# apache/arrow

Measured on AMD Instinct MI355X. Metric: filter_take_mrows_per_s, higher is better.
Workload: dtype int64; 1 GPU; Filter+Take int64[1000000000] + validity (10% null), boolean mask 10% true, FilterOptions::DROP; take indices = the mask's row numbers (monotonic; indices_nonzero: uint64 through CallFunction, GetTakeIndices: uint32 in the mirror), no boundscheck; inputs = splitmix64 streams of SURVEY.md 8(d) (seeds 1,2,3); rows=1000000000, selected_rows=99992053, parallelism=single-gpu

## Files before the change

arrow_amd/csrc/selection.hip:

```cpp
#include "arx_common.h"

#include <string.h>

#include <algorithm>
#include <type_traits>

namespace arx {

struct FilterWsHeader {
  int64_t total;
  int64_t ntiles;
  int64_t ngroups;
  int64_t length;
  int64_t valid;
  int64_t pad[3];
};
static_assert(sizeof(FilterWsHeader) == 64, "header is one 64-byte line");

struct FilterWsView {
  FilterWsHeader* hdr;
  int64_t* group_excl;
  int64_t* group_total;
  uint32_t* tile_counts;
  int64_t* group_valid;
};

static inline int64_t num_tiles(int64_t length) { return ceil_div(length, kTileRows); }
static inline int64_t num_groups(int64_t length) {
  return ceil_div(num_tiles(length), kTilesPerGroup);
}

static inline FilterWsView ws_view(void* ws, int64_t length) {
  FilterWsView v;
  const int64_t ng = num_groups(length);
  uint8_t* p = static_cast<uint8_t*>(ws);
  v.hdr = reinterpret_cast<FilterWsHeader*>(p);
  v.group_excl = reinterpret_cast<int64_t*>(p + 64);
  v.group_total = v.group_excl + ng;
  v.tile_counts = reinterpret_cast<uint32_t*>(v.group_total + ng);
  v.group_valid = reinterpret_cast<int64_t*>(v.tile_counts + ng * kTilesPerGroup);
  return v;
}

__device__ __forceinline__ uint64_t emit_word(const Bits& mask, const Bits& mvalid, int64_t w,
                                              bool emit_null, bool invert,
                                              uint64_t* mask_valid_out) {
  uint64_t m = load_word(mask, w);
  const uint64_t mv = load_word(mvalid, w);
  *mask_valid_out = mv;
  if (emit_null || invert) {
    const uint64_t in_range = load_word(Bits{nullptr, 0, mask.length, 0}, w);
    if (invert) m = ~m & in_range;
    if (emit_null) return (m | ~mv) & in_range;
  }
  return m & mv;
}

template <bool VALID>
__global__ __launch_bounds__(kBlock) void count_kernel(Bits mask, Bits mvalid, Bits vvalid, int emit_null,
                                                       int invert, int64_t ntiles,
                                                       uint32_t* tile_counts,
                                                       int64_t* group_total, int64_t* group_valid) {
  __shared__ uint32_t wave_sums[kWavesPerBlock];
  __shared__ uint32_t wave_valid[kWavesPerBlock];
  const int lane = lane_id();
  const int wave = threadIdx.x >> 6;
  const int64_t group = blockIdx.x;
  const int64_t t0 = group * kTilesPerGroup + wave * 16;
  uint32_t mine = 0;
  uint32_t kv = 0;
#pragma unroll 4
  for (int i = 0; i < 16; ++i) {
    const int64_t t = t0 + i;
    uint32_t k = 0;
    if (t < ntiles) {
      uint64_t mv;
      const uint64_t e = emit_word(mask, mvalid, t * 64 + lane, emit_null != 0, invert != 0, &mv);
      k = __popcll(e);
      if constexpr (VALID) kv += __popcll(e & mv & load_word(vvalid, t * 64 + lane));
    }
    const uint32_t s = wave_reduce_sum_u32(k);
    if (lane == i) mine = s;
  }
  if (lane < 16) tile_counts[t0 + lane] = mine;
  const uint32_t wsum = wave_reduce_sum_u32(lane < 16 ? mine : 0u);
  if (lane == 0) wave_sums[wave] = wsum;
  if constexpr (VALID) {
    const uint32_t vsum = wave_reduce_sum_u32(kv);
    if (lane == 0) wave_valid[wave] = vsum;
  }
  __syncthreads();
  if (threadIdx.x == 0) {
    int64_t s = 0, v = 0;
    for (int i = 0; i < kWavesPerBlock; ++i) {
      s += wave_sums[i];
      if constexpr (VALID) v += wave_valid[i];
    }
    group_total[group] = s;
    if constexpr (VALID) group_valid[group] = v;
  }
}

__global__ __launch_bounds__(1024) void scan_kernel(const int64_t* group_total, int64_t ngroups,
                                                    int64_t* group_excl, FilterWsHeader* hdr,
                                                    const int64_t* group_valid = nullptr) {
  __shared__ int64_t wave_tot[16];
  __shared__ int64_t carry_s;
  __shared__ unsigned long long valid_s;
  const int tid = threadIdx.x;
  const int lane = tid & 63;
  const int wave = tid >> 6;
  if (tid == 0) carry_s = 0;
  if (tid == 0) valid_s = 0;
  __syncthreads();
  if (group_valid != nullptr) {
    int64_t mine = 0;
    for (int64_t i = tid; i < ngroups; i += 1024) mine += group_valid[i];
#pragma unroll
    for (int d = 32; d >= 1; d >>= 1) mine += __shfl_xor(mine, d, 64);
    if (lane == 0 && mine != 0) atomicAdd(&valid_s, static_cast<unsigned long long>(mine));
    __syncthreads();
  }
  for (int64_t base = 0; base < ngroups; base += 1024) {
    const int64_t i = base + tid;
    const int64_t v = i < ngroups ? group_total[i] : 0;
    int64_t x = v;
#pragma unroll
    for (int d = 1; d < 64; d <<= 1) {
      const int64_t n = __shfl_up(x, d, 64);
      if (lane >= d) x += n;
    }
    if (lane == 63) wave_tot[wave] = x;
    __syncthreads();
    int64_t wave_prefix = 0;
    for (int k = 0; k < wave; ++k) wave_prefix += wave_tot[k];
    const int64_t carry = carry_s;
    if (i < ngroups) group_excl[i] = carry + wave_prefix + x - v;
    __syncthreads();
    if (tid == 1023) carry_s = carry + wave_prefix + x;
    __syncthreads();
  }
  if (tid == 0) {
    hdr->total = carry_s;
    hdr->valid = static_cast<int64_t>(valid_s);
  }
}

struct CompactArgs {
  const uint8_t* values;
  Bits mask;
  Bits mvalid;
  Bits vvalid;
  int64_t length;
  int64_t ntiles;
  const uint32_t* tile_counts;
  const int64_t* group_excl;
  uint8_t* out_data;
  uint64_t* out_validity;
  int emit_null;
  int invert;
  int values_aligned16;
};

constexpr int kFlushBytes = 2048;

template <int RING>
struct __attribute__((aligned(16))) CompactLds {
  uint8_t ring[kWavesPerBlock][RING];
  uint64_t vbits[kWavesPerBlock][72];
};

template <int W>
struct ElemT;
template <> struct ElemT<1> { using type = uint8_t; };
template <> struct ElemT<2> { using type = uint16_t; };
template <> struct ElemT<4> { using type = uint32_t; };
template <> struct ElemT<8> { using type = uint64_t; };
template <> struct ElemT<16> { using type = uint4; };
struct Elem32 { uint4 lo, hi; };
template <> struct ElemT<32> { using type = Elem32; };

template <int W>
__device__ __forceinline__ typename ElemT<W>::type zero_elem() {
  if constexpr (W == 32) {
    return Elem32{make_uint4(0, 0, 0, 0), make_uint4(0, 0, 0, 0)};
  } else if constexpr (W == 16) {
    return make_uint4(0, 0, 0, 0);
  } else {
    return 0;
  }
}

constexpr int kSelNt = 3;

template <int W>
__device__ __forceinline__ typename ElemT<W>::type sel_load(const typename ElemT<W>::type* p, bool nt) {
  using E = typename ElemT<W>::type;
  if constexpr (W == 32) {
    return *p;
  } else if constexpr (W == 16) {
    return nt ? nt_load16(p) : *p;
  } else {
    return nt ? nt_load<E>(p) : *p;
  }
}
template <int W>
__device__ __forceinline__ void sel_store(typename ElemT<W>::type* p, typename ElemT<W>::type v) {
  using E = typename ElemT<W>::type;
  if constexpr (W == 32) {
    *p = v;
  } else if constexpr (W == 16) {
    if constexpr ((kSelNt & 2) != 0) nt_store16(p, v); else *p = v;
  } else {
    if constexpr ((kSelNt & 2) != 0) nt_store<E>(p, v); else *p = v;
  }
}

__device__ __forceinline__ void wave_lds_sync() {
  __builtin_amdgcn_fence(__ATOMIC_RELEASE, "wavefront");
  __builtin_amdgcn_wave_barrier();
  __builtin_amdgcn_fence(__ATOMIC_ACQUIRE, "wavefront");
}

template <int W, int RING>
__device__ __forceinline__ void flush_region(const uint8_t* ring, uint8_t* gbase, int64_t F,
                                             int64_t lo, int64_t hi, int lane) {
  using E = typename ElemT<W>::type;
  constexpr int R = 16 / W;
  const int ring_off = static_cast<int>(F & (RING - 1));
#pragma unroll
  for (int h = 0; h < kFlushBytes / (16 * kWave); ++h) {
    const int g = h * kWave + lane;
    const int64_t gs = F + g * 16;
    const int64_t ge = gs + 16;
    if (ge <= lo || gs >= hi) continue;
    const uint8_t* src = ring + ring_off + g * 16;
    uint8_t* dst = gbase + gs;
    if (gs >= lo && ge <= hi) {
      sel_store<16>(reinterpret_cast<uint4*>(dst), *reinterpret_cast<const uint4*>(src));
    } else {
#pragma unroll
      for (int e = 0; e < R; ++e) {
        const int64_t es = gs + e * W;
        if (es >= lo && es + W <= hi) {
          *reinterpret_cast<E*>(dst + e * W) = *reinterpret_cast<const E*>(src + e * W);
        }
      }
    }
  }
}

template <int W, int B>
struct Batch {
  using E = typename ElemT<W>::type;
  static constexpr int R = 16 / W;
  uint32_t bits[B];
  uint32_t zbits[B];
  uint32_t rank[B];
  E v[B][R];
};

template <int R, bool EMIT>
__device__ __forceinline__ void select_words(uint64_t Ew, uint32_t p, uint64_t Zw,
                                             int widx_base, int lane, uint64_t* wE, uint32_t* wp,
                                             uint64_t* wZ) {
  constexpr int kLanesPerWord = 64 / R;
  const int q_mine = lane / kLanesPerWord;
  uint64_t e = 0, z = 0;
  uint32_t pp = 0;
#pragma unroll
  for (int q = 0; q < R; ++q) {
    const int src = widx_base + q;
    const uint32_t lo = __builtin_amdgcn_readlane(static_cast<uint32_t>(Ew), src);
    const uint32_t hi = __builtin_amdgcn_readlane(static_cast<uint32_t>(Ew >> 32), src);
    const uint32_t pq = __builtin_amdgcn_readlane(p, src);
    uint64_t zq = 0;
    if constexpr (EMIT) {
      const uint32_t zlo = __builtin_amdgcn_readlane(static_cast<uint32_t>(Zw), src);
      const uint32_t zhi = __builtin_amdgcn_readlane(static_cast<uint32_t>(Zw >> 32), src);
      zq = (static_cast<uint64_t>(zhi) << 32) | zlo;
    }
    if (q == q_mine) {
      e = (static_cast<uint64_t>(hi) << 32) | lo;
      pp = pq;
      z = zq;
    }
  }
  *wE = e;
  *wp = pp;
  *wZ = z;
}

struct TileCtx {
  uint64_t Ew, Zw;
  uint32_t p;
  int lane;
  int64_t tile_row0;
  const uint8_t* values;
  __amdgpu_buffer_rsrc_t rsrc;
};

template <int W, bool IOTA, bool EMIT, bool ALIGNED, int B>
__device__ __forceinline__ void issue_batch(const TileCtx& c, int j0, Batch<W, B>& b) {
  using E = typename ElemT<W>::type;
  constexpr int R = 16 / W;
  constexpr int kRowsPerIter = kWave * R;
#pragma unroll
  for (int i = 0; i < B; ++i) {
    const int j = j0 + i;
    const int row_in_tile = j * kRowsPerIter + c.lane * R;
    const int bpos = row_in_tile & 63;
    uint64_t wE, wZ;
    uint32_t wp;
    select_words<R, EMIT>(c.Ew, c.p, c.Zw, j * R, c.lane, &wE, &wp, &wZ);
    b.bits[i] = static_cast<uint32_t>(wE >> bpos) & ((1u << R) - 1u);
    b.zbits[i] = static_cast<uint32_t>(wZ >> bpos) & ((1u << R) - 1u);
    b.rank[i] = wp + __popcll(wE & low_mask64(bpos));
    if constexpr (IOTA) {
#pragma unroll
      for (int r = 0; r < R; ++r) b.v[i][r] = static_cast<E>(c.tile_row0 + row_in_tile + r);
    } else {
      const int64_t row = c.tile_row0 + row_in_tile;
      const uint8_t* src = c.values + row * static_cast<int64_t>(W);
      if constexpr (ALIGNED) {
        const uint32_t voff = b.bits[i] != 0 ? static_cast<uint32_t>(row_in_tile * W) : kBufferSkip;
        const uint4 q = (kSelNt & 1) ? buffer_load_b128_nt(c.rsrc, voff) : buffer_load_b128(c.rsrc, voff);
        if constexpr (W == 16) {
          b.v[i][0] = q;
        } else {
          const E* qe = reinterpret_cast<const E*>(&q);
#pragma unroll
          for (int r = 0; r < R; ++r) b.v[i][r] = qe[r];
        }
      } else {
#pragma unroll
        for (int r = 0; r < R; ++r) {
          b.v[i][r] = zero_elem<W>();
          if ((b.bits[i] >> r) & 1u) {
            if constexpr (W == 16) {
              const uint64_t* s64 = reinterpret_cast<const uint64_t*>(src + r * W);
              const uint64_t lo64 = s64[0], hi64 = s64[1];
              b.v[i][r] = make_uint4(static_cast<uint32_t>(lo64), static_cast<uint32_t>(lo64 >> 32),
                                     static_cast<uint32_t>(hi64), static_cast<uint32_t>(hi64 >> 32));
            } else {
              b.v[i][r] = *reinterpret_cast<const E*>(src + r * W);
            }
          }
        }
      }
    }
  }
}

template <int W, int B, int RING>
__device__ __forceinline__ void consume_batch(const Batch<W, B>& b, uint8_t* ring, int64_t a0) {
  using E = typename ElemT<W>::type;
  constexpr int R = 16 / W;
#pragma unroll
  for (int i = 0; i < B; ++i) {
    if (b.bits[i] != 0) {
      uint32_t rk = b.rank[i];
#pragma unroll
      for (int r = 0; r < R; ++r) {
        if ((b.bits[i] >> r) & 1u) {
          E e = b.v[i][r];
          if ((b.zbits[i] >> r) & 1u) e = zero_elem<W>();
          const int ro = static_cast<int>((a0 + static_cast<int64_t>(rk) * W) & (RING - 1));
          *reinterpret_cast<E*>(ring + ro) = e;
          ++rk;
        }
      }
    }
  }
}

template <int W, bool IOTA, bool EMIT, bool ALIGNED, int B, bool PIPE>
__global__ __launch_bounds__(kBlock) void compact_kernel(CompactArgs a) {
  using E = typename ElemT<W>::type;
  constexpr int R = 16 / W;
  constexpr int kRowsPerIter = kWave * R;
  constexpr int kIters = kTileRows / kRowsPerIter;
  constexpr int kWordsPerIter = kRowsPerIter / 64;
  constexpr int kBatches = kIters / B;
  constexpr int RING = (B <= 2) ? 4096 : 8192;
  static_assert(kIters % B == 0, "batch must divide the iteration count");
  static_assert(!PIPE || kBatches % 2 == 0, "pipelined form walks the batches in pairs");

  __shared__ CompactLds<RING> lds;

  const int lane = lane_id();
  const int wave = __builtin_amdgcn_readfirstlane(threadIdx.x >> 6);
  const int64_t t = static_cast<int64_t>(blockIdx.x) * kWavesPerBlock + wave;
  if (t >= a.ntiles) return;

  const int64_t w = t * 64 + lane;
  uint64_t mv;
  const uint64_t Ew = emit_word(a.mask, a.mvalid, w, EMIT, a.invert != 0, &mv);
  const uint32_t k = __popcll(Ew);
  const uint32_t incl = wave_inclusive_scan_u32(k);
  const uint32_t p = incl - k;
  const uint32_t total = __shfl(incl, 63, 64);
  if (total == 0) return;

  const int64_t grp = t >> 6;
  const int tin = static_cast<int>(t & 63);
  const uint32_t cprev = lane < tin ? a.tile_counts[grp * kTilesPerGroup + lane] : 0u;
  const int64_t off = a.group_excl[grp] + wave_reduce_sum_u32(cprev);

  uint8_t* ring = lds.ring[wave];
  const int64_t a0 =
      static_cast<int64_t>((reinterpret_cast<uint64_t>(a.out_data) + static_cast<uint64_t>(off) * W) &
                           (kFlushBytes - 1));
  uint8_t* gbase = a.out_data + (off * static_cast<int64_t>(W) - a0);
  int64_t flushed = 0;

  TileCtx c;
  c.Ew = Ew;
  c.Zw = EMIT ? (Ew & ~mv) : 0;
  c.p = p;
  c.lane = lane;
  c.tile_row0 = t * kTileRows;
  c.values = a.values;
  c.rsrc = make_rsrc(IOTA ? nullptr : a.values + c.tile_row0 * static_cast<int64_t>(W),
                     static_cast<uint32_t>(kTileRows * W));

  auto flush_check = [&](int next_batch) {
    const uint32_t cum = next_batch < kBatches
                             ? __builtin_amdgcn_readlane(p, next_batch * B * kWordsPerIter)
                             : total;
    const int64_t written = a0 + static_cast<int64_t>(cum) * W;
    if (written - flushed >= kFlushBytes) {
      wave_lds_sync();
      while (written - flushed >= kFlushBytes) {
        flush_region<W, RING>(ring, gbase, flushed, a0, written, lane);
        flushed += kFlushBytes;
      }
      wave_lds_sync();
    }
  };

  bool tile_done = false;
  if constexpr (IOTA) {
    if (a0 + static_cast<int64_t>(total) * W <= RING) {
      uint64_t m = Ew;
      uint32_t rk = p;
      while (m != 0) {
        const int bpos = __ffsll(static_cast<unsigned long long>(m)) - 1;
// ... 317 lines not shown
      }
    }
    E val[U];
#pragma unroll
    for (int u = 0; u < U; ++u) {
      const E* src = ok[u] ? (values + idx[u]) : (out + pos[u]);
      val[u] = sel_load<W>(src, (kSelNt & 4) != 0);
    }
    if constexpr (HAS_SV) {
      uint8_t vb[U];
#pragma unroll
      for (int u = 0; u < U; ++u) {
        const uint64_t bit = ok[u] ? static_cast<uint64_t>(a.src_valid_offset) + idx[u] : 0;
        vb[u] = a.src_valid_bytes[bit >> 3];
      }
#pragma unroll
      for (int u = 0; u < U; ++u) {
        const uint64_t bit = static_cast<uint64_t>(a.src_valid_offset) + idx[u];
        ok[u] = ok[u] && ((vb[u] >> (bit & 7)) & 1);
      }
    }
#pragma unroll
    for (int u = 0; u < U; ++u) {
      const int64_t p = base + u * 64 + lane;
      if (p <= last) sel_store<W>(out + p, ok[u] ? val[u] : zero_elem<W>());
      const uint64_t vbal = __ballot(ok[u]);
      nvalid += __popcll(vbal);
      if (a.out_validity != nullptr && lane == 0 && (base + u * 64) <= last) {
        a.out_validity[(base >> 6) + u] = vbal;
      }
    }
  }
  if (a.valid_count != nullptr && lane == 0 && nvalid != 0) atomicAdd(a.valid_count, nvalid);
}

template <int UB> struct RowUnit;
template <> struct RowUnit<1> { typedef uint8_t type; };
template <> struct RowUnit<2> { typedef uint16_t type; };
template <> struct RowUnit<4> { typedef uint32_t type; };
template <> struct RowUnit<8> { typedef uint64_t type; };
template <> struct RowUnit<16> { typedef arx_u32x4 type; };

template <int UB, typename IdxT, bool HAS_IV, bool HAS_SV>
__global__ __launch_bounds__(kBlock) void take_rows_kernel(TakeArgs a, uint32_t units_per_row) {
  using E = typename RowUnit<UB>::type;
  const int lane = lane_id();
  const int64_t nwaves = static_cast<int64_t>(gridDim.x) * kWavesPerBlock;
  const int64_t wave_g = static_cast<int64_t>(blockIdx.x) * kWavesPerBlock + __builtin_amdgcn_readfirstlane(threadIdx.x >> 6);
  const int64_t nchunks = (a.length + 63) >> 6;
  const int64_t last = a.length - 1;
  const IdxT* __restrict__ indices = reinterpret_cast<const IdxT*>(a.indices);
  const E* __restrict__ values = reinterpret_cast<const E*>(a.values);
  E* __restrict__ out = reinterpret_cast<E*>(a.out_data);
  uint64_t nvalid = 0;
  for (int64_t c = wave_g; c < nchunks; c += nwaves) {
    const int64_t base = c << 6;
    const int64_t p = base + lane <= last ? base + lane : last;
    uint64_t idx = static_cast<uint64_t>(indices[p]);
    bool ok = base + lane <= last;
    if constexpr (HAS_IV) ok = ok && ((load_word_nb(a.ivalid, base >> 6) >> lane) & 1ull);
    if constexpr (HAS_SV) {
      const uint64_t bit = ok ? static_cast<uint64_t>(a.src_valid_offset) + idx : 0;
      ok = ok && ((a.src_valid_bytes[bit >> 3] >> (bit & 7)) & 1);
    }
    if (!ok) idx = 0;
    const uint64_t vbal = __ballot(ok);
    nvalid += __popcll(vbal);
    if (a.out_validity != nullptr && lane == 0) a.out_validity[base >> 6] = vbal;
    const int rows_here = static_cast<int>(last - base + 1 < 64 ? last - base + 1 : 64);
    const uint32_t total = static_cast<uint32_t>(rows_here) * units_per_row;
    const uint32_t idx_lo = static_cast<uint32_t>(idx), idx_hi = static_cast<uint32_t>(idx >> 32);
    for (uint32_t t = lane; t < ((total + 63u) & ~63u); t += 64) {
      const uint32_t tt = t < total ? t : total - 1;
      const uint32_t row = tt / units_per_row;
      const uint32_t j = tt - row * units_per_row;
      const uint64_t src = (static_cast<uint64_t>(__shfl(idx_hi, static_cast<int>(row), 64)) << 32) | __shfl(idx_lo, static_cast<int>(row), 64);
      const bool row_ok = (vbal >> row) & 1ull;
      E v = E{};
      if (row_ok) v = values[src * units_per_row + j];
      if (t < total) out[(static_cast<uint64_t>(base) + row) * units_per_row + j] = v;
    }
  }
  if (a.valid_count != nullptr && lane == 0 && nvalid != 0) atomicAdd(a.valid_count, nvalid);
}

constexpr int kTakeMaxCols = 16;
struct TakeColsArgs {
  const uint8_t* values[kTakeMaxCols];
  const uint8_t* src_valid_bytes[kTakeMaxCols];
  int64_t src_valid_offset[kTakeMaxCols];
  uint8_t* out_data[kTakeMaxCols];
  uint64_t* out_validity[kTakeMaxCols];
  int width[kTakeMaxCols];
  int num_cols;
  const uint8_t* indices;
  Bits ivalid;
  int64_t length;
  unsigned long long* valid_counts;
};

template <int W, int U>
__device__ __forceinline__ uint64_t take_one_column(const TakeColsArgs& a, int c, const int64_t (&pos)[U],
                                                    const uint64_t (&idx)[U], const bool (&ok0)[U], int64_t base,
                                                    int64_t last, int lane) {
  using E = typename ElemT<W>::type;
  const E* __restrict__ values = reinterpret_cast<const E*>(a.values[c]);
  E* __restrict__ out = reinterpret_cast<E*>(a.out_data[c]);
  const uint8_t* __restrict__ svb = a.src_valid_bytes[c];
  const uint64_t svo = static_cast<uint64_t>(a.src_valid_offset[c]);
  E val[U];
  bool ok[U];
#pragma unroll
  for (int u = 0; u < U; ++u) {
    const E* src = ok0[u] ? (values + idx[u]) : (out + pos[u]);
    val[u] = *src;
    ok[u] = ok0[u];
  }
  if (svb != nullptr) {
    uint8_t vb[U];
#pragma unroll
    for (int u = 0; u < U; ++u) vb[u] = svb[(ok0[u] ? svo + idx[u] : 0) >> 3];
#pragma unroll
    for (int u = 0; u < U; ++u) ok[u] = ok[u] && ((vb[u] >> ((svo + idx[u]) & 7)) & 1);
  }
  uint64_t nvalid = 0;
#pragma unroll
  for (int u = 0; u < U; ++u) {
    const int64_t p = base + u * 64 + lane;
    if (p <= last) out[p] = ok[u] ? val[u] : zero_elem<W>();
    const uint64_t vbal = __ballot(ok[u]);
    nvalid += __popcll(vbal);
    if (a.out_validity[c] != nullptr && lane == 0 && (base + u * 64) <= last) a.out_validity[c][(base >> 6) + u] = vbal;
  }
  return nvalid;
}

template <typename IdxT, bool HAS_IV>
__global__ __launch_bounds__(kBlock) void take_columns_kernel(TakeColsArgs a) {
  constexpr int U = 4;
  const int lane = lane_id();
  const int64_t nwaves = static_cast<int64_t>(gridDim.x) * kWavesPerBlock;
  const int64_t wave_g = static_cast<int64_t>(blockIdx.x) * kWavesPerBlock +
                         __builtin_amdgcn_readfirstlane(threadIdx.x >> 6);
  const int64_t nchunks = (a.length + 64 * U - 1) / (64 * U);
  const int64_t last = a.length - 1;
  const IdxT* __restrict__ indices = reinterpret_cast<const IdxT*>(a.indices);
  uint64_t nvalid[kTakeMaxCols];
  for (int c = 0; c < kTakeMaxCols; ++c) nvalid[c] = 0;
  for (int64_t ch = wave_g; ch < nchunks; ch += nwaves) {
    const int64_t base = ch * (64 * U);
    int64_t pos[U];
    uint64_t idx[U];
    bool ok0[U];
#pragma unroll
    for (int u = 0; u < U; ++u) {
      const int64_t p = base + u * 64 + lane;
      pos[u] = p <= last ? p : last;
      idx[u] = static_cast<uint64_t>(indices[pos[u]]);
    }
#pragma unroll
    for (int u = 0; u < U; ++u) {
      ok0[u] = (base + u * 64 + lane) <= last;
      if constexpr (HAS_IV) {
        const uint64_t wbits = load_word_nb(a.ivalid, (base >> 6) + u);
        ok0[u] = ok0[u] && ((wbits >> lane) & 1ull);
      }
    }
    for (int c = 0; c < a.num_cols; ++c) {
      uint64_t nv;
      switch (a.width[c]) {
        case 1: nv = take_one_column<1, U>(a, c, pos, idx, ok0, base, last, lane); break;
        case 2: nv = take_one_column<2, U>(a, c, pos, idx, ok0, base, last, lane); break;
        case 4: nv = take_one_column<4, U>(a, c, pos, idx, ok0, base, last, lane); break;
        case 8: nv = take_one_column<8, U>(a, c, pos, idx, ok0, base, last, lane); break;
        case 16: nv = take_one_column<16, U>(a, c, pos, idx, ok0, base, last, lane); break;
        default: nv = take_one_column<32, U>(a, c, pos, idx, ok0, base, last, lane); break;
      }
      nvalid[c] += nv;
    }
  }
  if (a.valid_counts != nullptr && lane == 0) {
    for (int c = 0; c < a.num_cols; ++c) {
      if (nvalid[c] != 0) atomicAdd(a.valid_counts + c, nvalid[c]);
    }
  }
}

template <typename IdxT>
__global__ __launch_bounds__(kBlock) void take_bits_kernel(TakeArgs a, int64_t value_bit_offset) {
  const int lane = lane_id();
  const int64_t nwaves = static_cast<int64_t>(gridDim.x) * kWavesPerBlock;
  const int64_t wave_g = static_cast<int64_t>(blockIdx.x) * kWavesPerBlock +
                         __builtin_amdgcn_readfirstlane(threadIdx.x >> 6);
  const int64_t nwords = (a.length + 63) >> 6;
  const int64_t last = a.length - 1;
  const IdxT* __restrict__ indices = reinterpret_cast<const IdxT*>(a.indices);
  uint64_t* __restrict__ out = reinterpret_cast<uint64_t*>(a.out_data);
  uint64_t nvalid = 0;
  for (int64_t w = wave_g; w < nwords; w += nwaves) {
    const int64_t p = (w << 6) + lane;
    const int64_t pc = p <= last ? p : last;
    const uint64_t idx = static_cast<uint64_t>(indices[pc]);
    bool ok = p <= last && ((load_word(a.ivalid, w) >> lane) & 1ull);
    if (ok && a.src_valid_bytes != nullptr) {
      const uint64_t vb = static_cast<uint64_t>(a.src_valid_offset) + idx;
      ok = (a.src_valid_bytes[vb >> 3] >> (vb & 7)) & 1;
    }
    bool bit = false;
    if (ok) {
      const uint64_t b = static_cast<uint64_t>(value_bit_offset) + idx;
      bit = (a.values[b >> 3] >> (b & 7)) & 1;
    }
    const uint64_t data_bal = __ballot(bit);
    const uint64_t valid_bal = __ballot(ok);
    nvalid += __popcll(valid_bal);
    if (lane == 0) {
      out[w] = data_bal;
      if (a.out_validity != nullptr) a.out_validity[w] = valid_bal;
    }
  }
  if (a.valid_count != nullptr && lane == 0 && nvalid != 0) atomicAdd(a.valid_count, nvalid);
}

struct BoundsWs {
  unsigned long long first_bad_pos;
  long long bad_value_signed;
  unsigned long long bad_value_unsigned;
  int64_t pad[5];
};

template <typename IdxT>
__global__ __launch_bounds__(kBlock) void bounds_kernel(const uint8_t* indices, Bits ivalid,
                                                        int64_t length, uint64_t upper,
                                                        BoundsWs* ws) {
  const int64_t stride = static_cast<int64_t>(gridDim.x) * blockDim.x;
  unsigned long long bad = ~0ull;
  for (int64_t i = static_cast<int64_t>(blockIdx.x) * blockDim.x + threadIdx.x; i < length;
       i += stride) {
    const IdxT v = reinterpret_cast<const IdxT*>(indices)[i];
    const bool valid = (load_word(ivalid, i >> 6) >> (i & 63)) & 1ull;
    bool oob;
    if constexpr (std::is_signed<IdxT>::value) {
      oob = v < 0 || static_cast<uint64_t>(v) >= upper;
    } else {
      oob = static_cast<uint64_t>(v) >= upper;
    }
    if (valid && oob) {
      bad = static_cast<unsigned long long>(i);
      break;
    }
  }
  if (bad != ~0ull) atomicMin(&ws->first_bad_pos, bad);
}

template <typename IdxT>
__global__ void bounds_fetch_kernel(const uint8_t* indices, BoundsWs* ws) {
  const unsigned long long pos = ws->first_bad_pos;
  if (pos == ~0ull) return;
  const IdxT v = reinterpret_cast<const IdxT*>(indices)[pos];
  ws->bad_value_signed = static_cast<long long>(v);
  ws->bad_value_unsigned = static_cast<unsigned long long>(v);
}

static int check_mask(const ArxSpan* mask, int null_selection) {
  if (mask == nullptr) {
    set_error("filter mask is NULL");
    return ARX_INVALID;
  }
  if (mask->length < 0 || mask->offset < 0) {
    set_error("negative length/offset");
    return ARX_INVALID;
  }
  if (mask->length > 0 && mask->data == nullptr) {
    set_error("filter mask has no data buffer");
    return ARX_INVALID;
  }
  if (null_selection != ARX_FILTER_DROP && null_selection != ARX_FILTER_EMIT_NULL) {
    set_error("bad null_selection %d", null_selection);
    return ARX_INVALID;
  }
  return ARX_OK;
}

static inline const void* effective_validity(const ArxSpan* s) {
  return (s->null_count != 0) ? s->validity : nullptr;
}

static int launch_count(const ArxSpan* mask, int null_selection, void* ws, size_t ws_bytes,
                        hipStream_t st, int invert = 0, const ArxSpan* values = nullptr) {
  const int rc = check_mask(mask, null_selection);
  if (rc != ARX_OK) return rc;
  const size_t need = arx_filter_workspace_bytes(mask->length);
  if (ws == nullptr || ws_bytes < need) {
    set_error("filter workspace too small: %zu < %zu", ws_bytes, need);
    return ARX_INVALID;
  }
  if ((reinterpret_cast<uint64_t>(ws) & 63) != 0) {
    set_error("filter workspace must be 64-byte aligned");
    return ARX_INVALID;
  }
  FilterWsView v = ws_view(ws, mask->length);
  const int64_t nt = num_tiles(mask->length);
  const int64_t ng = num_groups(mask->length);
  FilterWsHeader h{};
  h.total = 0;
  h.ntiles = nt;
  h.ngroups = ng;
  h.length = mask->length;
  ARX_HIP(hipMemcpyAsync(v.hdr, &h, sizeof(h), hipMemcpyHostToDevice, st));
  if (mask->length == 0) return ARX_OK;
  const Bits mb = make_bits(mask->data, mask->offset, mask->length);
  const Bits mvb = make_bits(effective_validity(mask), mask->offset, mask->length);
  if (values != nullptr) {
    const Bits vvb = make_bits(effective_validity(values), values->offset, mask->length);
    hipLaunchKernelGGL((count_kernel<true>), dim3(static_cast<unsigned>(ng)), dim3(kBlock), 0, st, mb, mvb, vvb,
                       null_selection, invert, nt, v.tile_counts, v.group_total, v.group_valid);
    ARX_CHECK_LAUNCH("count_kernel");
    hipLaunchKernelGGL(scan_kernel, dim3(1), dim3(1024), 0, st, v.group_total, ng, v.group_excl, v.hdr,
                       static_cast<const int64_t*>(v.group_valid));
  } else {
    hipLaunchKernelGGL((count_kernel<false>), dim3(static_cast<unsigned>(ng)), dim3(kBlock), 0, st, mb, mvb, mvb,
                       null_selection, invert, nt, v.tile_counts, v.group_total, static_cast<int64_t*>(nullptr));
    ARX_CHECK_LAUNCH("count_kernel");
    hipLaunchKernelGGL(scan_kernel, dim3(1), dim3(1024), 0, st, v.group_total, ng, v.group_excl, v.hdr,
                       static_cast<const int64_t*>(nullptr));
  }
  ARX_CHECK_LAUNCH("scan_kernel");
  return ARX_OK;
}

static Knob<int> g_filter_batch{4};
static Knob<int> g_filter_pipe{1};
static Knob<int> g_filter_sparse{-1};
static const KnobRow kSelectionKnobs[] = {
    {"filter_batch", g_filter_batch, knob_snap_down<1, 4>},
    {"filter_pipe", g_filter_pipe, knob_bool},
    {"filter_sparse", g_filter_sparse, knob_tri},
};
KnobTable selection_knobs() { return knob_table(kSelectionKnobs); }

template <int W, bool IOTA, bool EMIT, bool ALIGNED>
static void launch_compact_e(const CompactArgs& a, unsigned grid, hipStream_t st) {
  constexpr int kIters = kTileRows / (kWave * (16 / W));
  constexpr int kBig = kIters >= 8 ? 4 : 2;
  if (ALIGNED && g_filter_batch >= 4 && g_filter_pipe) {
    hipLaunchKernelGGL((compact_kernel<W, IOTA, EMIT, ALIGNED, kBig, true>), dim3(grid),
                       dim3(kBlock), 0, st, a);
  } else {
    hipLaunchKernelGGL((compact_kernel<W, IOTA, EMIT, ALIGNED, 1, false>), dim3(grid), dim3(kBlock),
                       0, st, a);
  }
}

template <int W, bool IOTA>
static void launch_compact_w(const CompactArgs& a, unsigned grid, hipStream_t st) {
  const bool aligned = IOTA || a.values_aligned16 != 0;
  if (a.emit_null) {
    if (aligned) launch_compact_e<W, IOTA, true, true>(a, grid, st);
    else if constexpr (!IOTA) launch_compact_e<W, IOTA, true, false>(a, grid, st);
  } else {
    if (aligned) launch_compact_e<W, IOTA, false, true>(a, grid, st);
    else if constexpr (!IOTA) launch_compact_e<W, IOTA, false, false>(a, grid, st);
  }
}

template <int W, bool IOTA = false>
static void launch_sparse_w(const CompactArgs& a, unsigned grid, hipStream_t st) {
  if (a.emit_null) {
    hipLaunchKernelGGL((compact_sparse_kernel<W, true, IOTA>), dim3(grid), dim3(kBlock), 0, st, a);
  } else {
    hipLaunchKernelGGL((compact_sparse_kernel<W, false, IOTA>), dim3(grid), dim3(kBlock), 0, st, a);
  }
}

static int launch_compact(bool iota, int W, const CompactArgs& a, hipStream_t st,
                          int64_t out_length = -1) {
  const unsigned grid = static_cast<unsigned>(ceil_div(a.ntiles, kWavesPerBlock));
  const int filter_sparse = g_filter_sparse;
  const bool sparse = !iota && !a.invert &&
                      (filter_sparse == 1 ||
                       (filter_sparse < 0 &&
                        (W >= 8 || (out_length >= 0 && out_length * 4 <= a.length))));
  if (iota && !a.invert && filter_sparse != 0 && (W == 2 || W == 4 || W == 8)) {
    if (W == 2) launch_sparse_w<2, true>(a, grid, st);
    else if (W == 4) launch_sparse_w<4, true>(a, grid, st);
    else launch_sparse_w<8, true>(a, grid, st);
    ARX_CHECK_LAUNCH("compact_sparse_kernel<IOTA>");
    return ARX_OK;
  }
  if (sparse) {
    switch (W) {
      case 1: launch_sparse_w<1>(a, grid, st); break;
      case 2: launch_sparse_w<2>(a, grid, st); break;
      case 4: launch_sparse_w<4>(a, grid, st); break;
      case 8: launch_sparse_w<8>(a, grid, st); break;
      case 16: launch_sparse_w<16>(a, grid, st); break;
      case 32: launch_sparse_w<32>(a, grid, st); break;
      default:
        set_error("unsupported byte width %d for the gfx950 filter", W);
        return ARX_NOT_IMPLEMENTED;
    }
    ARX_CHECK_LAUNCH("compact_sparse_kernel");
    return ARX_OK;
  }
  if (iota) {
    switch (W) {
      case 2: launch_compact_w<2, true>(a, grid, st); break;
      case 4: launch_compact_w<4, true>(a, grid, st); break;
      default:
        set_error("unsupported index width %d", W);
        return ARX_NOT_IMPLEMENTED;
    }
  } else {
    switch (W) {
      case 1: launch_compact_w<1, false>(a, grid, st); break;
      case 2: launch_compact_w<2, false>(a, grid, st); break;
      case 4: launch_compact_w<4, false>(a, grid, st); break;
      case 8: launch_compact_w<8, false>(a, grid, st); break;
      case 16: launch_compact_w<16, false>(a, grid, st); break;
      default:
        set_error("unsupported byte width %d for the gfx950 filter", W);
        return ARX_NOT_IMPLEMENTED;
    }
  }
  ARX_CHECK_LAUNCH("compact_kernel");
  return ARX_OK;
}

static int zero_out_validity(void* out_validity, int64_t out_length, hipStream_t st) {
  if (out_validity == nullptr) return ARX_OK;
  if ((reinterpret_cast<uint64_t>(out_validity) & 7) != 0) {
    set_error("out_validity must be 8-byte aligned");
    return ARX_INVALID;
  }
  if (out_length < 0) {
    set_error("out_length (from arx_filter_count) is required when out_validity is given");
    return ARX_INVALID;
  }
  if (out_length > 0) {
    ARX_HIP(hipMemsetAsync(out_validity, 0, static_cast<size_t>(ceil_div(out_length, 64)) * 8, st));
  }
  return ARX_OK;
}

size_t selection_workspace_bytes(int64_t length) { return arx_filter_workspace_bytes(length); }

int selection_bit_positions(const void* bitmap, int64_t bit_offset, int64_t length, bool invert,
                            void* ws, size_t ws_bytes, uint32_t* out, int64_t* out_count_host,
                            hipStream_t st) {
  ArxSpan m{};
  m.validity = nullptr;
  m.data = bitmap;
  m.offset = bit_offset;
  m.length = length;
  m.null_count = 0;
  int rc = launch_count(&m, ARX_FILTER_DROP, ws, ws_bytes, st, invert ? 1 : 0);
  if (rc != ARX_OK) return rc;
  int64_t total = 0;
  ARX_HIP(hipMemcpyAsync(&total, ws, sizeof(int64_t), hipMemcpyDeviceToHost, st));
  ARX_HIP(hipStreamSynchronize(st));
  *out_count_host = total;
  if (total == 0) return ARX_OK;
  FilterWsView v = ws_view(ws, length);
  CompactArgs a{};
  a.values = nullptr;
  a.mask = make_bits(bitmap, bit_offset, length);
  a.mvalid = make_bits(nullptr, 0, length);
  a.vvalid = make_bits(nullptr, 0, length);
  a.length = length;
  a.ntiles = num_tiles(length);
  a.tile_counts = v.tile_counts;
  a.group_excl = v.group_excl;
  a.out_data = reinterpret_cast<uint8_t*>(out);
  a.out_validity = nullptr;
  a.emit_null = 0;
  a.invert = invert ? 1 : 0;
  a.values_aligned16 = 1;
  return launch_compact(true, 4, a, st);
}

}

using namespace arx;

extern "C" {

size_t arx_filter_workspace_bytes(int64_t length) {
  if (length < 0) length = 0;
  const int64_t ng = num_groups(length);
  return static_cast<size_t>(64 + ng * 16 + ng * kTilesPerGroup * 4 + ng * 8 + 64);
}

int arx_filter_count_async(const ArxSpan* mask, int null_selection, void* ws, size_t ws_bytes,
                           void* stream) {
  return launch_count(mask, null_selection, ws, ws_bytes, as_stream(stream));
}

int arx_filter_count_nulls(const ArxSpan* values, const ArxSpan* mask, int null_selection, void* ws, size_t ws_bytes,
                           int64_t* out_length, int64_t* out_null_count, void* stream) {
  if (out_length == nullptr || out_null_count == nullptr || values == nullptr) {
    set_error("values / out_length / out_null_count is NULL");
    return ARX_INVALID;
  }
  if (mask != nullptr && values->length != mask->length) {
    set_error("filter values and mask differ in length (%lld vs %lld)", static_cast<long long>(values->length),
              static_cast<long long>(mask->length));
    return ARX_INVALID;
  }
  hipStream_t st = as_stream(stream);
  const int rc = launch_count(mask, null_selection, ws, ws_bytes, st, 0, values);
  if (rc != ARX_OK) return rc;
  int64_t hdr[5] = {0, 0, 0, 0, 0};
  ARX_HIP(hipMemcpyAsync(hdr, ws, sizeof(hdr), hipMemcpyDeviceToHost, st));
  ARX_HIP(hipStreamSynchronize(st));
  *out_length = hdr[0];
  *out_null_count = mask->length == 0 ? 0 : hdr[0] - hdr[4];
  return ARX_OK;
}

int arx_filter_count(const ArxSpan* mask, int null_selection, void* ws, size_t ws_bytes,
                     int64_t* out_length, void* stream) {
  if (out_length == nullptr) {
    set_error("out_length is NULL");
    return ARX_INVALID;
  }
  hipStream_t st = as_stream(stream);
  const int rc = launch_count(mask, null_selection, ws, ws_bytes, st);
  if (rc != ARX_OK) return rc;
  int64_t total = 0;
  ARX_HIP(hipMemcpyAsync(&total, ws, sizeof(int64_t), hipMemcpyDeviceToHost, st));
  ARX_HIP(hipStreamSynchronize(st));
  *out_length = total;
  return ARX_OK;
}

int arx_filter_exec(const ArxSpan* values, int byte_width, const ArxSpan* mask, int null_selection,
                    const void* ws, int64_t out_length, void* out_data, void* out_validity,
                    void* stream) {
  int rc = check_mask(mask, null_selection);
  if (rc != ARX_OK) return rc;
  if (values == nullptr || ws == nullptr) {
    set_error("values/ws is NULL");
    return ARX_INVALID;
  }
  if (values->length != mask->length) {
    set_error("Array arguments must all be the same length (values %lld vs filter %lld)",
              static_cast<long long>(values->length), static_cast<long long>(mask->length));
    return ARX_INVALID;
  }
  if (mask->length == 0) return ARX_OK;
  if (values->data == nullptr || out_data == nullptr) {
    set_error("values/out data buffer is NULL");
    return ARX_INVALID;
  }
  hipStream_t st = as_stream(stream);
  FilterWsView v = ws_view(const_cast<void*>(ws), mask->length);
  CompactArgs a{};
  a.values = static_cast<const uint8_t*>(values->data) + values->offset * byte_width;
  a.mask = make_bits(mask->data, mask->offset, mask->length);
  a.mvalid = make_bits(effective_validity(mask), mask->offset, mask->length);
  a.vvalid = make_bits(effective_validity(values), values->offset, values->length);
  a.length = mask->length;
  a.ntiles = num_tiles(mask->length);
  a.tile_counts = v.tile_counts;
  a.group_excl = v.group_excl;
  a.out_data = static_cast<uint8_t*>(out_data);
  a.out_validity = static_cast<uint64_t*>(out_validity);
  a.emit_null = null_selection == ARX_FILTER_EMIT_NULL && a.mvalid.base != nullptr;
  a.values_aligned16 = (reinterpret_cast<uint64_t>(a.values) & 15) == 0;
  if ((reinterpret_cast<uint64_t>(out_data) % byte_width) != 0) {
    set_error("out_data is not aligned to the element width");
    return ARX_INVALID;
  }
  rc = zero_out_validity(out_validity, out_length, st);
  if (rc != ARX_OK) return rc;
  return launch_compact(false, byte_width, a, st, out_length);
}

int arx_expand_by_mask(const void* dense, int byte_width, const ArxSpan* mask, const void* ws, void* out_data,
                       void* stream) {
  int rc = check_mask(mask, ARX_FILTER_DROP);
  if (rc != ARX_OK) return rc;
  if (ws == nullptr) {
    set_error("ws is NULL (run arx_filter_count on the mask first)");
    return ARX_INVALID;
  }
  if (mask->length == 0) return ARX_OK;
  if (out_data == nullptr || (reinterpret_cast<uint64_t>(out_data) % byte_width) != 0 ||
      (dense != nullptr && (reinterpret_cast<uint64_t>(dense) % byte_width) != 0)) {
    set_error("expand: NULL or misaligned buffer");
    return ARX_INVALID;
  }
  FilterWsView v = ws_view(const_cast<void*>(ws), mask->length);
  CompactArgs a{};
  a.values = static_cast<const uint8_t*>(dense);
  a.mask = make_bits(mask->data, mask->offset, mask->length);
  a.mvalid = make_bits(effective_validity(mask), mask->offset, mask->length);
  a.length = mask->length;
  a.ntiles = num_tiles(mask->length);
  a.tile_counts = v.tile_counts;
  a.group_excl = v.group_excl;
  a.out_data = static_cast<uint8_t*>(out_data);
  const unsigned grid = static_cast<unsigned>(ceil_div(a.ntiles, kWavesPerBlock));
  hipStream_t st = as_stream(stream);
  switch (byte_width) {
    case 1: hipLaunchKernelGGL((expand_kernel<1>), dim3(grid), dim3(kBlock), 0, st, a); break;
    case 2: hipLaunchKernelGGL((expand_kernel<2>), dim3(grid), dim3(kBlock), 0, st, a); break;
    case 4: hipLaunchKernelGGL((expand_kernel<4>), dim3(grid), dim3(kBlock), 0, st, a); break;
    case 8: hipLaunchKernelGGL((expand_kernel<8>), dim3(grid), dim3(kBlock), 0, st, a); break;
    case 16: hipLaunchKernelGGL((expand_kernel<16>), dim3(grid), dim3(kBlock), 0, st, a); break;
    default:
      set_error("unsupported byte width %d for expand", byte_width);
      return ARX_NOT_IMPLEMENTED;
  }
  ARX_CHECK_LAUNCH("expand_kernel");
  return ARX_OK;
}

int arx_mask_to_indices(const ArxSpan* mask, int null_selection, const void* ws, int64_t out_length,
                        int index_width, void* out_indices, void* out_validity, void* stream) {
  int rc = check_mask(mask, null_selection);
  if (rc != ARX_OK) return rc;
  if (ws == nullptr) {
    set_error("ws is NULL");
    return ARX_INVALID;
  }
  if (index_width != 2 && index_width != 4 && index_width != 8) {
    set_error("index_width must be 2, 4 or 8");
// ... 389 lines not shown
```

Measured before the change: 291,300 Mrows/s.

## Batch count-kernel bitmap loads up front and drop host header memcpy

The count kernel now issues every bitmap word load for a wave's 16 tiles up front into registers, using an aligned fast path when no shifts are present and a shifted two-word path otherwise. It falls back to per-word loads near the buffer end. It also packs two tile popcounts into a single wave reduction, and adds a launch-bounds occupancy hint. The host-to-device header memcpy is removed; the scan kernel now writes the full header itself, which saves an async copy on the stream. The cost is higher register pressure from the preloaded arrays.

After: 293,900 Mrows/s, median of 6. Within noise of the previous version (+0.9%).

```diff
diff --git a/arrow_amd/csrc/selection.hip b/arrow_amd/csrc/selection.hip
--- a/arrow_amd/csrc/selection.hip
+++ b/arrow_amd/csrc/selection.hip
@@ -42,25 +42,92 @@
   return v;
 }
 
+__device__ __forceinline__ uint64_t emit_combine(int64_t length, int64_t w, uint64_t m, uint64_t mv,
+                                                 bool emit_null, bool invert) {
+  if (emit_null || invert) {
+    const uint64_t in_range = load_word(Bits{nullptr, 0, length, 0}, w);
+    if (invert) m = ~m & in_range;
+    if (emit_null) return (m | ~mv) & in_range;
+  }
+  return m & mv;
+}
+
 __device__ __forceinline__ uint64_t emit_word(const Bits& mask, const Bits& mvalid, int64_t w,
                                               bool emit_null, bool invert,
                                               uint64_t* mask_valid_out) {
-  uint64_t m = load_word(mask, w);
+  const uint64_t m = load_word(mask, w);
   const uint64_t mv = load_word(mvalid, w);
   *mask_valid_out = mv;
-  if (emit_null || invert) {
-    const uint64_t in_range = load_word(Bits{nullptr, 0, mask.length, 0}, w);
-    if (invert) m = ~m & in_range;
-    if (emit_null) return (m | ~mv) & in_range;
-  }
-  return m & mv;
+  return emit_combine(mask.length, w, m, mv, emit_null, invert);
+}
+
+struct RawWord {
+  uint64_t lo, hi;
+};
+__device__ __forceinline__ uint64_t finish_word(const Bits& b, int64_t w, const RawWord& r) {
+  const int64_t remain = b.length - (w << 6);
+  if (remain <= 0) return 0;
+  uint64_t v = ~uint64_t(0);
+  if (b.base != nullptr) v = (r.lo >> b.shift) | ((r.hi << 1) << (63 - b.shift));
+  if (remain < 64) v &= low_mask64(static_cast<int>(remain));
+  return v;
+}
+
+template <bool VALID, int ROWS, bool SHIFTED>
+__device__ __forceinline__ void count_rows(const Bits& mask, const Bits& mvalid, const Bits& vvalid, bool emit_null,
+                                           bool invert, int64_t t0, int lane, uint32_t* mine, uint32_t* kv) {
+  constexpr int NB = VALID ? 3 : 2;
+  const Bits* bits[3] = {&mask, &mvalid, &vvalid};
+  const int l0 = static_cast<int>(t0 & 15);
+  const int64_t last_word = (t0 + ROWS) * 64 - 1 + (SHIFTED ? 1 : 0);
+  bool inside = true;
+#pragma unroll
+  for (int b = 0; b < NB; ++b) inside = inside && (bits[b]->base == nullptr || last_word < bits[b]->nphys);
+  if (!inside) {
+    for (int i = 0; i < ROWS; ++i) {
+      const int64_t w = (t0 + i) * 64 + lane;
+      uint64_t mv;
+      const uint64_t e = emit_word(mask, mvalid, w, emit_null, invert, &mv);
+      if constexpr (VALID) *kv += __popcll(e & mv & load_word(vvalid, w));
+      const uint32_t s = wave_reduce_sum_u32(__popcll(e));
+      if (lane == l0 + i) *mine = s;
+    }
+    return;
+  }
+  uint64_t lo[3][ROWS] = {}, hi[3][ROWS] = {};
+#pragma unroll
+  for (int b = 0; b < NB; ++b) {
+    if (bits[b]->base == nullptr) continue;
+    const uint64_t* __restrict__ p = bits[b]->base + t0 * 64;
+#pragma unroll
+    for (int i = 0; i < ROWS; ++i) {
+      lo[b][i] = p[static_cast<uint32_t>(lane + 64 * i)];
+      if constexpr (SHIFTED) hi[b][i] = p[static_cast<uint32_t>(lane + 64 * i + 1)];
+    }
+  }
+#pragma unroll
+  for (int i = 0; i < ROWS; i += 2) {
+    uint32_t k2 = 0;
+#pragma unroll
+    for (int h = 0; h < 2; ++h) {
+      const int64_t w = (t0 + i + h) * 64 + lane;
+      const uint64_t m = finish_word(mask, w, RawWord{lo[0][i + h], hi[0][i + h]});
+      const uint64_t mv = finish_word(mvalid, w, RawWord{lo[1][i + h], hi[1][i + h]});
+      const uint64_t e = emit_combine(mask.length, w, m, mv, emit_null, invert);
+      k2 |= static_cast<uint32_t>(__popcll(e)) << (16 * h);
+      if constexpr (VALID) *kv += __popcll(e & mv & finish_word(vvalid, w, RawWord{lo[2][i + h], hi[2][i + h]}));
+    }
+    const uint32_t s = wave_reduce_sum_u32(k2);
+    if (lane == l0 + i) *mine = s & 0xffffu;
+    if (lane == l0 + i + 1) *mine = s >> 16;
+  }
 }
 
 template <bool VALID>
-__global__ __launch_bounds__(kBlock) void count_kernel(Bits mask, Bits mvalid, Bits vvalid, int emit_null,
-                                                       int invert, int64_t ntiles,
-                                                       uint32_t* tile_counts,
-                                                       int64_t* group_total, int64_t* group_valid) {
+__global__ __launch_bounds__(kBlock, 4) void count_kernel(Bits mask, Bits mvalid, Bits vvalid, int emit_null,
+                                                          int invert, int64_t ntiles,
+                                                          uint32_t* tile_counts,
+                                                          int64_t* group_total, int64_t* group_valid) {
   __shared__ uint32_t wave_sums[kWavesPerBlock];
   __shared__ uint32_t wave_valid[kWavesPerBlock];
   const int lane = lane_id();
@@ -69,18 +136,12 @@
   const int64_t t0 = group * kTilesPerGroup + wave * 16;
   uint32_t mine = 0;
   uint32_t kv = 0;
-#pragma unroll 4
-  for (int i = 0; i < 16; ++i) {
-    const int64_t t = t0 + i;
-    uint32_t k = 0;
-    if (t < ntiles) {
-      uint64_t mv;
-      const uint64_t e = emit_word(mask, mvalid, t * 64 + lane, emit_null != 0, invert != 0, &mv);
-      k = __popcll(e);
-      if constexpr (VALID) kv += __popcll(e & mv & load_word(vvalid, t * 64 + lane));
-    }
-    const uint32_t s = wave_reduce_sum_u32(k);
-    if (lane == i) mine = s;
+  const bool en = emit_null != 0, inv = invert != 0;
+  if ((mask.shift | mvalid.shift | (VALID ? vvalid.shift : 0)) == 0) {
+    count_rows<VALID, 16, false>(mask, mvalid, vvalid, en, inv, t0, lane, &mine, &kv);
+  } else {
+    count_rows<VALID, 8, true>(mask, mvalid, vvalid, en, inv, t0, lane, &mine, &kv);
+    count_rows<VALID, 8, true>(mask, mvalid, vvalid, en, inv, t0 + 8, lane, &mine, &kv);
   }
   if (lane < 16) tile_counts[t0 + lane] = mine;
   const uint32_t wsum = wave_reduce_sum_u32(lane < 16 ? mine : 0u);
@@ -103,6 +164,7 @@
 
 __global__ __launch_bounds__(1024) void scan_kernel(const int64_t* group_total, int64_t ngroups,
                                                     int64_t* group_excl, FilterWsHeader* hdr,
+                                                    int64_t ntiles, int64_t length,
                                                     const int64_t* group_valid = nullptr) {
   __shared__ int64_t wave_tot[16];
   __shared__ int64_t carry_s;
@@ -141,8 +203,13 @@
     __syncthreads();
   }
   if (tid == 0) {
-    hdr->total = carry_s;
-    hdr->valid = static_cast<int64_t>(valid_s);
+    FilterWsHeader h{};
+    h.total = carry_s;
+    h.ntiles = ntiles;
+    h.ngroups = ngroups;
+    h.length = length;
+    h.valid = static_cast<int64_t>(valid_s);
+    *hdr = h;
   }
 }
 
@@ -1066,13 +1133,11 @@
   FilterWsView v = ws_view(ws, mask->length);
   const int64_t nt = num_tiles(mask->length);
   const int64_t ng = num_groups(mask->length);
-  FilterWsHeader h{};
-  h.total = 0;
-  h.ntiles = nt;
-  h.ngroups = ng;
-  h.length = mask->length;
-  ARX_HIP(hipMemcpyAsync(v.hdr, &h, sizeof(h), hipMemcpyHostToDevice, st));
-  if (mask->length == 0) return ARX_OK;
+  if (mask->length == 0) {
+    const FilterWsHeader h{};
+    ARX_HIP(hipMemcpyAsync(v.hdr, &h, sizeof(h), hipMemcpyHostToDevice, st));
+    return ARX_OK;
+  }
   const Bits mb = make_bits(mask->data, mask->offset, mask->length);
   const Bits mvb = make_bits(effective_validity(mask), mask->offset, mask->length);
   if (values != nullptr) {
@@ -1080,14 +1145,14 @@
     hipLaunchKernelGGL((count_kernel<true>), dim3(static_cast<unsigned>(ng)), dim3(kBlock), 0, st, mb, mvb, vvb,
                        null_selection, invert, nt, v.tile_counts, v.group_total, v.group_valid);
     ARX_CHECK_LAUNCH("count_kernel");
-    hipLaunchKernelGGL(scan_kernel, dim3(1), dim3(1024), 0, st, v.group_total, ng, v.group_excl, v.hdr,
-                       static_cast<const int64_t*>(v.group_valid));
+    hipLaunchKernelGGL(scan_kernel, dim3(1), dim3(1024), 0, st, v.group_total, ng, v.group_excl, v.hdr, nt,
+                       mask->length, static_cast<const int64_t*>(v.group_valid));
   } else {
     hipLaunchKernelGGL((count_kernel<false>), dim3(static_cast<unsigned>(ng)), dim3(kBlock), 0, st, mb, mvb, mvb,
                        null_selection, invert, nt, v.tile_counts, v.group_total, static_cast<int64_t*>(nullptr));
     ARX_CHECK_LAUNCH("count_kernel");
-    hipLaunchKernelGGL(scan_kernel, dim3(1), dim3(1024), 0, st, v.group_total, ng, v.group_excl, v.hdr,
-                       static_cast<const int64_t*>(nullptr));
+    hipLaunchKernelGGL(scan_kernel, dim3(1), dim3(1024), 0, st, v.group_total, ng, v.group_excl, v.hdr, nt,
+                       mask->length, static_cast<const int64_t*>(nullptr));
   }
   ARX_CHECK_LAUNCH("scan_kernel");
   return ARX_OK;
```
